# GeoMop/MLMC

Hardware: AMD Instinct MI355X
Metric: moment-evals/sec (samples x n_moments) (higher is better)
Workload: dtype f64

## Files before the change

### mlmc_amd/csrc/api.hip

```cpp
#include <cmath>
#include <chrono>
#include <cstring>
#include <new>

#include "common.hpp"
#include <algorithm>
#include <map>
#include <tuple>

namespace mlmc {

static thread_local std::string g_err;
void set_error(const std::string &msg) { g_err = msg; }
int fail(const std::string &msg) {
    g_err = msg;
    return 1;
}
Runtime &rt() {
    static Runtime r;
    return r;
}
std::recursive_mutex &api_mutex() {
    static std::recursive_mutex m;
    return m;
// ... 596 lines not shown
    return rc;
}

int mlmc_accum_create(const mlmc_basis *b, int32_t n_levels, int32_t mode, int32_t n_comp, mlmc_accum **out) {
    MLMC_API_GUARD;
    if (need_runtime()) return 1;
    if (!b || !out) return fail("mlmc_accum_create: null argument");
    if (n_levels <= 0 || n_comp <= 0) return fail("mlmc_accum_create: n_levels and n_comp must be > 0");
    const bool mean_only = (mode & MLMC_MODE_MEAN_ONLY) != 0;
    mode &= ~MLMC_MODE_MEAN_ONLY;
    if (mode != MLMC_MODE_MOMENTS && mode != MLMC_MODE_COV) return fail("mlmc_accum_create: unknown mode");
    mlmc_accum *a = new (std::nothrow) mlmc_accum();
    if (!a) return fail("out of memory");
    a->basis = b;
    a->n_levels = n_levels;
    a->mode = mode;
    const bool spline_band = mode == MLMC_MODE_COV && mean_only && b->out_size == 0 && b->p.kind == MLMC_SPLINE && b->p.size <= SPLINE_BAND_MAX_R;
    a->cov_from_values = mode == MLMC_MODE_COV && (b->out_size > 0 || (b->p.size > 128 && !spline_band));
    a->mean_only = mean_only && ((mode == MLMC_MODE_COV && !a->cov_from_values) || (mode == MLMC_MODE_MOMENTS && b->out_size > 0));
    a->mean_only_plain = mean_only && mode == MLMC_MODE_MOMENTS && b->out_size == 0 &&
                         (b->p.kind == MLMC_LEGENDRE || b->p.kind == MLMC_MONOMIAL || b->p.kind == KIND_CHEBYSHEV) && b->p.size > 64 &&
                         b->p.size <= 256;
    a->n_comp = n_comp;
    a->R = b->p.size;
    a->Rout = b->out_size > 0 ? b->out_size : b->p.size;
    a->RP = (((mode == MLMC_MODE_COV && b->out_size > 0 ? a->Rout : a->R) + 15) / 16) * 16;
    if (mode == MLMC_MODE_MOMENTS) {
        a->K = (int64_t)n_comp * a->Rout;
        a->int_width = 2 * (int64_t)a->R + (b->out_size > 0 ? (int64_t)a->RP * a->RP : 0);
    } else {
        a->K = (int64_t)n_comp * a->Rout * a->Rout;
        a->int_width = 3 * (int64_t)a->RP * a->RP;
    }
    const size_t tot = (size_t)n_levels * n_comp * a->int_width;
    a->state_bytes = sizeof(double) * tot + sizeof(int64_t) * 2 * n_levels;
    a->out_bytes = (sizeof(int64_t) + sizeof(double)) * 2 * n_levels + 2 * sizeof(double) * (size_t)n_levels * a->K;
    if (hipMalloc(&a->d_state, a->state_bytes) != hipSuccess || hipMalloc(&a->d_out, a->out_bytes) != hipSuccess ||
        hipHostMalloc(&a->h_out, a->out_bytes, hipHostMallocDefault) != hipSuccess) {
        mlmc_accum_destroy(a);
        return fail("mlmc_accum_create: device / pinned allocation failed");
    }
    a->d_totals = (double *)a->d_state;
    a->d_counts = (int64_t *)(a->d_totals + tot);
    a->level_flushed.assign(n_levels, 0);
    if (mode == MLMC_MODE_MOMENTS && n_comp == 1 && b->out_size == 0) {
        void *dev_view = nullptr;
// ... 11 lines not shown
    if (mode == MLMC_MODE_COV && !mean_only && !a->cov_from_values && b->out_size == 0 && b->p.size > lin_min_size() && b->p.size <= 128 &&
        (b->p.kind == MLMC_LEGENDRE || b->p.kind == MLMC_MONOMIAL) && b->p.is_clip &&
        std::fabs(b->p.ref0) <= 1.0 && std::fabs(b->p.ref1) <= 1.0 &&
        linearize_enabled()) {
        a->lin_eligible = true;
        const char *min_n = std::getenv("MLMC_HIP_LINEARIZE_MIN_N");
        a->lin_min_n = min_n ? std::atoll(min_n) : (a->R > 32 ? 100000 : 1500000);
        const char *lin0_env = std::getenv("MLMC_HIP_LINEARIZE_LEVEL0");
        a->lin0_eligible = a->R <= 64 && !(lin0_env && lin0_env[0] == '0');
        a->lin_cheb = b->p.kind == MLMC_LEGENDRE && linearize_chebyshev_enabled() && std::getenv("MLMC_HIP_NO_SPLIT") == nullptr;
        a->cov_rows = a->lin_cheb && a->lin0_eligible && a->R >= 49 && a->R <= 64 && a->RP == 64 && linearize_rowsums_enabled() &&
                      cov_rows_available();
    }
    *out = a;
    return mlmc_accum_reset(a);
}

int mlmc_accum_reset(mlmc_accum *a) {
    MLMC_API_GUARD;
    if (need_runtime()) return 1;
    if (!a) return fail("mlmc_accum_reset: null argument");
    hipStream_t st = rt().stream;
    a->pending.clear();
    std::fill(a->level_flushed.begin(), a->level_flushed.end(), 0);
    MLMC_HIP_CHECK(hipMemsetAsync(a->d_state, 0, a->state_bytes, st));
    if (a->xcov) {
        MLMC_HIP_CHECK(hipMemcpyAsync(a->d_shift, a->shift_host.data(), sizeof(double) * a->shift_host.size(), hipMemcpyHostToDevice, st));
        a->xcov_pushes = 0;
    }
    a->lin_used = a->lin0_used = false;
    if (a->d_rowsums) MLMC_HIP_CHECK(hipMemsetAsync(a->d_rowsums, 0, sizeof(double) * 64 * (size_t)a->n_levels * a->n_comp, st));
    a->lin_levels.assign(a->n_levels, 0);
    a->lin0_levels.assign(a->n_levels, 0);
    if (a->lin0)
        if (int rc = mlmc_accum_reset(a->lin0)) return rc;
    if (a->lin) return mlmc_accum_reset(a->lin);
    return 0;
}

void mlmc_accum_destroy(mlmc_accum *a) {
    MLMC_API_GUARD;
    if (!a) return;
    if (rt().ready) (void)wait_stream(rt().stream);
    if (a->lin) mlmc_accum_destroy(a->lin);
    if (a->lin_basis) mlmc_basis_destroy(a->lin_basis);
    if (a->lin0) mlmc_accum_destroy(a->lin0);
    if (a->lin0_basis) mlmc_basis_destroy(a->lin0_basis);
    void *ptrs[] = {a->d_state, a->d_partials, a->d_pcounts, a->d_stage_f, a->d_stage_c, a->d_mask, a->d_out, a->d_vals_f, a->d_vals_c, a->d_vals_tmp,
                    a->d_shift, a->d_rowparts, a->d_rowsums};
    for (void *p : ptrs)
        if (p) (void)hipFree(p);
    if (a->h_out) (void)hipHostFree(a->h_out);
    for (hipEvent_t e : a->ev) (void)hipEventDestroy(e);
    delete a;
}

int mlmc_accum_push(mlmc_accum *a, int32_t level, const double *fine, const double *coarse, int64_t n, int mem_kind) {
    MLMC_API_GUARD;
    if (need_runtime()) return 1;
    if (!a) return fail("mlmc_accum_push: null argument");
    if (level < 0 || level >= a->n_levels) return fail("mlmc_accum_push: level out of range");
    if (n < 0) return fail("mlmc_accum_push: negative n");
    if (n == 0) return 0;
    if (!fine) return fail("mlmc_accum_push: fine is NULL");
    if (n > ((int64_t)1 << 40)) return fail("mlmc_accum_push: chunk too large, split it");
    hipStream_t st = rt().stream;
    const size_t bytes = sizeof(double) * (size_t)n * a->n_comp;
    const double *d_f = fine, *d_c = coarse;
    if (mem_kind == MLMC_HOST) {
        if (bytes > a->stage_cap) {
            MLMC_HIP_CHECK(wait_stream(st));
            if (a->d_stage_f) (void)hipFree(a->d_stage_f);
            if (a->d_stage_c) (void)hipFree(a->d_stage_c);
            a->d_stage_f = a->d_stage_c = nullptr;
// ... 348 lines not shown
```

### mlmc_amd/csrc/common.hpp

```cpp
#pragma once
#include <hip/hip_runtime.h>
#include <stdint.h>
#include <mutex>
#include <string>
#include <vector>

#include "../../include/mlmc_hip.h"

namespace mlmc {

constexpr int WAVE = 64;
constexpr int ACC_THREADS = 256;
#ifndef MLMC_TERMS_PER_PASS
#define MLMC_TERMS_PER_PASS 64
#endif
constexpr int MAX_TERMS_PER_PASS = MLMC_TERMS_PER_PASS;
constexpr int KIND_CHEBYSHEV = 16;
static_assert(KIND_CHEBYSHEV > MLMC_SPLINE && KIND_CHEBYSHEV > MLMC_IDENTITY && KIND_CHEBYSHEV > MLMC_FOURIER && KIND_CHEBYSHEV > MLMC_MONOMIAL &&
                  KIND_CHEBYSHEV > MLMC_LEGENDRE && KIND_CHEBYSHEV > 7,
              "KIND_CHEBYSHEV must not collide with a public basis kind of mlmc_hip.h");
constexpr int SPLINE_BAND_MAX_R = 256;

void set_error(const std::string &msg);
int fail(const std::string &msg);
#define MLMC_HIP_CHECK(expr)                                                                   \
    do {                                                                                       \
        hipError_t _e = (expr);                                                                \
        if (_e != hipSuccess)                                                                  \
            return ::mlmc::fail(std::string(#expr) + ": " + hipGetErrorString(_e));            \
    } while (0)

std::recursive_mutex &api_mutex();
void bind_thread_to_device();
struct ApiGuard {
    std::lock_guard<std::recursive_mutex> lock;
    ApiGuard() : lock(api_mutex()) { bind_thread_to_device(); }
};
#define MLMC_API_GUARD ::mlmc::ApiGuard mlmc_api_guard_

struct Runtime {
    bool ready = false;
    int device = -1;
    int flags = 0;
// ... 31 lines not shown
    const uint64_t p0 = (uint64_t)0xD2511F53u * c[0], p1 = (uint64_t)0xCD9E8D57u * c[2];
    const uint32_t n0 = (uint32_t)(p1 >> 32) ^ c[1] ^ k0, n1 = (uint32_t)p1;
    const uint32_t n2 = (uint32_t)(p0 >> 32) ^ c[3] ^ k1, n3 = (uint32_t)p0;
    c[0] = n0; c[1] = n1; c[2] = n2; c[3] = n3;
}

struct BasisParams {
    int kind;
    int size;
    double shift, scale, ref0, ref1;
    int is_log, is_clip;
    double x_lo, x_hi;
};

}

struct mlmc_basis {
    mlmc::BasisParams p;
    int out_size = 0;
    std::vector<double> matrix;
    std::vector<double> scale_c;
    double *d_scale = nullptr;
    double *d_matrix = nullptr;
};

struct PendingSeg {
    const double *fine, *coarse;
    const uint8_t *mask;
    int64_t n;
    int level, comp;
    bool count;
};

struct mlmc_accum {
    const mlmc_basis *basis = nullptr;
    int n_levels = 0, mode = 0, n_comp = 1;
    bool mean_only = false;
    bool cov_from_values = false;
    bool mean_only_plain = false;
    int R = 0;
    int Rout = 0;
    int64_t K = 0;
    int64_t int_width = 0;
    void *d_state = nullptr;
    size_t state_bytes = 0;
    double *d_totals = nullptr;
    int64_t *d_counts = nullptr;
    double *d_partials = nullptr; size_t partials_cap = 0;
    int64_t *d_pcounts = nullptr; size_t pcounts_cap = 0;
    double *d_stage_f = nullptr, *d_stage_c = nullptr; size_t stage_cap = 0;
    uint8_t *d_mask = nullptr; size_t mask_cap = 0;
    double *d_vals_f = nullptr, *d_vals_c = nullptr; size_t vals_cap = 0;
    double *d_vals_tmp = nullptr; size_t vals_tmp_cap = 0;
    void *d_out = nullptr;
    size_t out_bytes = 0;
    void *h_out = nullptr;
    bool host_outputs = false;
    double *packed_target = nullptr;
    double *h_out_s = nullptr, *h_out_sp = nullptr; int64_t *h_out_n = nullptr;
    std::vector<char> level_flushed;
    double *d_out_s = nullptr, *d_out_sp = nullptr, *d_out_nd = nullptr; int64_t *d_out_n = nullptr;
    std::vector<hipEvent_t> ev;
    size_t ev_used = 0;
    double ms_total = 0;
    int64_t launches = 0, alg_bytes = 0;
    int64_t mfma_flops = 0;
    int RP = 0;
    bool lin_eligible = false, lin0_eligible = false;
    mlmc_accum *lin = nullptr;
    mlmc_basis *lin_basis = nullptr;
    double *d_lin_prod = nullptr;
    int lin_K = 0;
// ... 10 lines not shown
    bool cov_rows = false;
    double *d_rowparts = nullptr; size_t rowparts_cap = 0;
    double *d_rowsums = nullptr;
    double *d_conn = nullptr;
    int first_term = 0;
    std::vector<PendingSeg> pending;
    bool xcov = false;
    double *d_shift = nullptr;
    std::vector<double> shift_host;
    int64_t xcov_pushes = 0;
};

namespace mlmc {
int launch_eval(const mlmc_basis *b, const double *d_x, int64_t n, int size, double *d_out, double *scratch = nullptr);
int launch_eval_scaled_base(const mlmc_basis *b, const double *d_x, int64_t n, double *d_out);
int launch_mask(const mlmc_accum *a, const double *d_f, const double *d_c, int64_t n, uint8_t *d_mask, int64_t *d_counts_level);
int launch_moments_accum(mlmc_accum *a, int level, int comp, const double *d_f, const double *d_c, const uint8_t *d_mask,
                         int64_t n, bool count, bool defer);
int flush_moments(mlmc_accum *a);
int launch_moments_finalize(mlmc_accum *a);
int launch_cov_accum(mlmc_accum *a, int level, int comp, const double *d_f, const double *d_c, const uint8_t *d_mask,
                     int64_t n, bool count, int gram_mode, int ncomp = 1);
int launch_cov_finalize(mlmc_accum *a);
bool cov_rows_available();
constexpr int XCOV_MAX_M = 1024;
constexpr int MODE_XCOV = 2;
int launch_xcov_push(mlmc_accum *a, int level, const double *d_f, const double *d_c, int64_t n);
int launch_xcov_finalize(mlmc_accum *a);
bool product_table(int kind, int R, std::vector<double> &out);
bool square_product_table(int kind, int R, std::vector<double> &out);
bool product_table_chebyshev(int R, std::vector<double> &out);
bool square_product_table_chebyshev(int R, std::vector<double> &out);
int launch_cov_from_values(mlmc_accum *a, int level, int comp, const double *d_vf, const double *d_vc, const uint8_t *d_mask,
                           int64_t n, bool count, int gram_mode = 0);
int ensure(void **p, size_t *cap, size_t bytes);
void gauss_legendre(int n, std::vector<double> &x, std::vector<double> &w);
std::vector<double> effective_coeffs(const mlmc_basis *b, const double *lambda, const double *sigma, int R1);
int timing_begin(mlmc_accum *a);
int timing_end(mlmc_accum *a);
}
```

### mlmc_amd/csrc/cov.hip

```cpp
#include <cstring>

#include "device_basis.hpp"

namespace mlmc {

typedef double v4f64 __attribute__((ext_vector_type(4)));
#ifdef MLMC_PROF_COV
__device__ unsigned long long *g_prof_cov;
#define MLMC_COV_STAMP(slot)                                      \
    {                                                             \
        const unsigned long long now_ = __builtin_amdgcn_s_memtime(); \
        prof_acc[slot] += now_ - prof_t;                          \
        prof_t = now_;                                            \
    }
#else
#define MLMC_COV_STAMP(slot)
#endif
#ifndef MLMC_COV_PRIO_MFMA
#define MLMC_COV_PRIO_MFMA 0
#define MLMC_COV_PRIO_EVAL 2
#endif
#ifndef MLMC_COV_SLICE_BITS
#define MLMC_COV_SLICE_BITS 17
#endif
// ... 684 lines not shown
#define MLMC_COV_HAVE_ROWS 1
template <int KIND>
__global__ __launch_bounds__(256, COV_T4_WGS) void k_cov_accum_t4_rows(BasisParams bp, const double *__restrict__ fine,
                                                              const double *__restrict__ coarse, const uint8_t *__restrict__ mask,
                                                              int64_t n, double *__restrict__ partials,
                                                              int64_t *__restrict__ pcounts, double *__restrict__ rowparts) {
    __shared__ __attribute__((aligned(16))) double lds_f[64 * (COV_T4_BATCH + MLMC_COV_B128_PAD)];
    __shared__ __attribute__((aligned(16))) double lds_c[64 * (COV_T4_BATCH + MLMC_COV_B128_PAD)];
    __shared__ int ldc[2][2];
    fine += (int64_t)blockIdx.y * n;
    coarse += (int64_t)blockIdx.y * n;
    partials += (int64_t)blockIdx.y * gridDim.x * (cov_ng(3) * 64 * 64);
    rowparts += (int64_t)blockIdx.y * gridDim.x * 64;
    if (blockIdx.y) pcounts = nullptr;
    switch (__builtin_amdgcn_readfirstlane((int)(threadIdx.x >> 6))) {
        case 0: cov_t4_body<KIND, true, 3, 0, 0, true>(bp, fine, coarse, mask, n, partials, pcounts, lds_f, lds_c, ldc, rowparts); break;
        case 1: cov_t4_body<KIND, true, 3, 0, 1, true>(bp, fine, coarse, mask, n, partials, pcounts, lds_f, lds_c, ldc, rowparts); break;
        case 2: cov_t4_body<KIND, true, 3, 0, 2, true>(bp, fine, coarse, mask, n, partials, pcounts, lds_f, lds_c, ldc, rowparts); break;
        default: cov_t4_body<KIND, true, 3, 0, 3, true>(bp, fine, coarse, mask, n, partials, pcounts, lds_f, lds_c, ldc, rowparts); break;
    }
}
#endif

__global__ __launch_bounds__(1024) void k_reduce_cov(const double *__restrict__ partials, int nrows, int NT, int NG, int RP,
                                                    int roff, int coff, double *__restrict__ totals, int64_t comp_stride,
                                                    int mirror, const int64_t *__restrict__ pcounts, int nblocks,
                                                    int64_t *__restrict__ counts, const double *__restrict__ rowparts = nullptr,
                                                    double *__restrict__ rowsums = nullptr) {
    __shared__ double lds[64][17];
    const int c = threadIdx.x & 15, g = threadIdx.x >> 4;
    const int width = NG * NT * NT;
    const int n_col_groups = (width + 15) / 16;
    if (rowparts && (int)blockIdx.x >= n_col_groups && (int)blockIdx.x < n_col_groups + 4) {
        const int col = ((int)blockIdx.x - n_col_groups) * 16 + c;
        rowparts += (int64_t)blockIdx.y * nrows * 64;
        double acc = 0.0;
        for (int b = g; b < nrows; b += 64) acc += rowparts[(int64_t)b * 64 + col];
        lds[g][c] = acc;
        __syncthreads();
        if (g == 0) {
            double v = 0.0;
#pragma unroll
            for (int k = 0; k < 64; ++k) v += lds[k][c];
            rowsums[(int64_t)blockIdx.y * 64 + col] += v;
        }
        return;
    }
    if (pcounts && blockIdx.x == gridDim.x - 1) {
        if (blockIdx.y == 0 && threadIdx.x < 64) {
            int64_t a = 0, b = 0;
            for (int i = threadIdx.x; i < nblocks; i += 64) { a += pcounts[2 * i]; b += pcounts[2 * i + 1]; }
            for (int off = 32; off >= 1; off >>= 1) { a += __shfl_xor(a, off, 64); b += __shfl_xor(b, off, 64); }
            if (threadIdx.x == 0) { counts[0] += a; counts[1] += b; }
        }
        return;
    }
    partials += (int64_t)blockIdx.y * nrows * width;
    totals += (int64_t)blockIdx.y * comp_stride;
    const int col = blockIdx.x * 16 + c;
    double acc = 0.0;
    if (col < width)
        for (int b = g; b < nrows; b += 64) acc += partials[(int64_t)b * width + col];
    lds[g][c] = acc;
    __syncthreads();
    if (g == 0 && col < width) {
        double v = 0.0;
#pragma unroll
        for (int k = 0; k < 64; ++k) v += lds[k][c];
        const int gi = col / (NT * NT), rem = col % (NT * NT);
        const int row = roff + rem / NT, cc = coff + rem % NT;
        if (row < RP && cc < RP) {
            totals[(int64_t)gi * RP * RP + (int64_t)row * RP + cc] += v;
            if (mirror) totals[(int64_t)gi * RP * RP + (int64_t)cc * RP + row] += v;
        }
    }
}

template <int KIND, int T, int MODE, int BI, int BJ>
static int launch_cov_t(const BasisParams &bp, bool pair, int blocks, int ncomp, const double *d_f, const double *d_c,
                        const uint8_t *d_mask, int64_t n, int R, double *partials, int64_t *pcounts) {
    hipStream_t st = rt().stream;
    if constexpr (T == 4 && BI == BJ) {
        if (pair)
            hipLaunchKernelGGL((k_cov_accum_t4<KIND, true, MODE, BI>), dim3(blocks, ncomp), dim3(256), 0, st, bp, d_f, d_c, d_mask, n, R, partials, pcounts);
        else
            hipLaunchKernelGGL((k_cov_accum_t4<KIND, false, MODE, BI>), dim3(blocks, ncomp), dim3(256), 0, st, bp, d_f, d_c, d_mask, n, R, partials, pcounts);
    } else {
        if (pair)
            hipLaunchKernelGGL((k_cov_accum<KIND, T, true, MODE, BI, BJ>), dim3(blocks, ncomp), dim3(256), 0, st, bp, d_f, d_c, d_mask, n, R, partials, pcounts, 0, 0);
        else
            hipLaunchKernelGGL((k_cov_accum<KIND, T, false, MODE, BI, BJ>), dim3(blocks, ncomp), dim3(256), 0, st, bp, d_f, d_c, d_mask, n, R, partials, pcounts, 0, 0);
    }
    MLMC_HIP_CHECK(hipGetLastError());
    return 0;
}

template <int KIND, int MODE>
static int launch_cov_kind(const BasisParams &bp, int T, int bi, int bj, bool pair, int blocks, int ncomp, const double *d_f,
// ... 12 lines not shown
int launch_cov_from_values(mlmc_accum *a, int level, int comp, const double *d_vf, const double *d_vc, const uint8_t *d_mask,
                           int64_t n, bool count, int gram_mode) {
    if (n == 0) return 0;
    const bool diff_gram = gram_mode == 1;
    const int R = diff_gram ? a->R : a->Rout;
    hipStream_t st = rt().stream;
    const int T = (R <= 16) ? 1 : (R <= 32 ? 2 : 4);
    const int NT = 16 * T, NSL = 4 / T;
    const bool pair = d_vc != nullptr;
    const int NB = (R + 63) / 64;
    const int64_t n_batches = (n + COV_BATCH - 1) / COV_BATCH;
    const int NG = diff_gram ? 1 : 3;
    const size_t width = (size_t)NG * NT * NT;
    const BasisParams &bp = a->basis->p;
    double *totals = a->d_totals + ((int64_t)level * a->n_comp + comp) * a->int_width + (diff_gram ? 2 * (int64_t)R : 0);
    const bool symmetric = !pair || diff_gram;
    for (int bi = 0; bi < NB; ++bi)
        for (int bj = 0; bj < NB; ++bj) {
            if (symmetric && bj < bi) continue;
            const bool wide = bi != bj;
            int blocks = rt().n_cu * (wide ? 1 : 2);
            if (n_batches < blocks) blocks = (int)n_batches;
            const int n_slices = T <= 2 ? 4 : NSL;
            if (int rc = ensure((void **)&a->d_partials, &a->partials_cap, sizeof(double) * (size_t)blocks * n_slices * width)) return rc;
            if (int rc = ensure((void **)&a->d_pcounts, &a->pcounts_cap, sizeof(int64_t) * (size_t)blocks * 2)) return rc;
            const bool do_count = count && bi == 0 && bj == 0 && !diff_gram;
            int64_t *pc = do_count ? a->d_pcounts : nullptr;
            if (int rc = timing_begin(a)) return rc;
#define MLMC_COV_VALS1(TT, BJJ, MODE)                                                                                           \
    do {                                                                                                                        \
        if (pair)                                                                                                               \
            hipLaunchKernelGGL((k_cov_accum<MLMC_IDENTITY, TT, true, MODE, 0, BJJ, true>), dim3(blocks), dim3(256), 0, st, bp,      \
                               d_vf, d_vc, d_mask, n, R, a->d_partials, pc, 64 * bi, 64 * bj);                                  \
        else                                                                                                                    \
            hipLaunchKernelGGL((k_cov_accum<MLMC_IDENTITY, TT, false, MODE, 0, BJJ, true>), dim3(blocks), dim3(256), 0, st, bp,     \
                               d_vf, d_vc, d_mask, n, R, a->d_partials, pc, 64 * bi, 64 * bj);                                  \
    } while (0)
#define MLMC_COV_VALS(TT, BJJ)                                                                                                  \
    do {                                                                                                                        \
        if (diff_gram) MLMC_COV_VALS1(TT, BJJ, 1); else MLMC_COV_VALS1(TT, BJJ, 0);                                             \
    } while (0)
            if (T == 1) MLMC_COV_VALS(1, 0);
            else if (T == 2) MLMC_COV_VALS(2, 0);
            else if (!wide) MLMC_COV_VALS(4, 0);
            else MLMC_COV_VALS(4, 1);
#undef MLMC_COV_VALS
#undef MLMC_COV_VALS1
            MLMC_HIP_CHECK(hipGetLastError());
            if (int rc = timing_end(a)) return rc;
            if (!diff_gram) {
                a->launches += 1;
                a->alg_bytes += (int64_t)n * (pair ? 16 : 8);
                a->mfma_flops += (int64_t)512 * n * (T <= 2 ? (pair ? 2 * T * T + T * (T + 1) / 2 : T * (T + 1)) : (pair ? 3 : 2) * 16);
            }
            hipLaunchKernelGGL(k_reduce_cov, dim3((unsigned)((width + 15) / 16) + (do_count ? 1u : 0u)), dim3(1024), 0, st, a->d_partials,
                               blocks * n_slices, NT, NG, a->RP, 64 * bi, 64 * bj, totals, (int64_t)0, (symmetric && wide) ? 1 : 0,
                               do_count ? a->d_pcounts : (const int64_t *)nullptr, blocks, a->d_counts + 2 * (int64_t)level);
            MLMC_HIP_CHECK(hipGetLastError());
        }
    return 0;
}

constexpr int BAND_W = 5;
template <bool PAIR>
__global__ __launch_bounds__(256) void k_spline_band_accum(BasisParams bp, const double *__restrict__ fine,
                                                          const double *__restrict__ coarse, const uint8_t *__restrict__ mask,
                                                          int64_t n, int R, double *__restrict__ partials,
                                                          int64_t *__restrict__ pcounts) {
    extern __shared__ double band_tab[];
    __shared__ int ldc[4][2];
    const int RP8 = R + 8;
    fine += (int64_t)blockIdx.y * n;
    if (PAIR) coarse += (int64_t)blockIdx.y * n;
    partials += (int64_t)blockIdx.y * gridDim.x * (BAND_W * R);
    if (blockIdx.y) pcounts = nullptr;
    const int lane = threadIdx.x & 63, wave = threadIdx.x >> 6;
    for (int i = threadIdx.x; i < 4 * RP8 * BAND_W; i += 256) band_tab[i] = 0.0;
    __syncthreads();
    double *__restrict__ tab = band_tab + (size_t)wave * RP8 * BAND_W;
    int n_keep = 0, n_rm = 0;
    const int64_t T = (int64_t)gridDim.x * 256;
// ... 83 lines not shown
    __syncthreads();
    if (g == 0 && col < width) {
        double v = 0.0;
#pragma unroll
        for (int k = 0; k < 64; ++k) v += lds[k][c];
        const int r = col / BAND_W, w = col % BAND_W;
        if (r >= 1) {
            if (w == 4) {
                totals[r] += v;
                totals[(int64_t)r * RP] += v;
            } else if (r + w < R) {
                totals[(int64_t)r * RP + r + w] += v;
                if (w) totals[(int64_t)(r + w) * RP + r] += v;
            }
        }
    }
}

static int launch_spline_band(mlmc_accum *a, int level, int comp, const double *d_f, const double *d_c, const uint8_t *d_mask, int64_t n,
                              bool count, int ncomp) {
    hipStream_t st = rt().stream;
    const int R = a->R;
    const bool pair = d_c != nullptr;
    int blocks = rt().n_cu * 4;
    const int64_t want = (n + 255) / 256;
    if (want < blocks) blocks = (int)want;
    if (int rc = ensure((void **)&a->d_partials, &a->partials_cap, sizeof(double) * (size_t)blocks * BAND_W * R * ncomp)) return rc;
    if (int rc = ensure((void **)&a->d_pcounts, &a->pcounts_cap, sizeof(int64_t) * (size_t)blocks * 2)) return rc;
    const size_t lds = sizeof(double) * 4 * (size_t)(R + 8) * BAND_W;
    const BasisParams &bp = a->basis->p;
    double *totals = a->d_totals + ((int64_t)level * a->n_comp + comp) * a->int_width;
    if (int rc = timing_begin(a)) return rc;
    if (pair)
        hipLaunchKernelGGL(k_spline_band_accum<true>, dim3(blocks, ncomp), dim3(256), lds, st, bp, d_f, d_c, d_mask, n, R, a->d_partials, a->d_pcounts);
    else
        hipLaunchKernelGGL(k_spline_band_accum<false>, dim3(blocks, ncomp), dim3(256), lds, st, bp, d_f, d_c, d_mask, n, R, a->d_partials, a->d_pcounts);
    MLMC_HIP_CHECK(hipGetLastError());
    if (int rc = timing_end(a)) return rc;
    a->launches += 1;
    a->alg_bytes += (int64_t)n * (pair ? 16 : 8) * ncomp;
    hipLaunchKernelGGL(k_reduce_band, dim3((BAND_W * R + 15) / 16 + 1, ncomp), dim3(1024), 0, st, a->d_partials, a->d_pcounts, blocks, R, a->RP,
                       totals, a->int_width, count ? a->d_counts + 2 * (int64_t)level : (int64_t *)nullptr, pair ? 0 : 1);
    MLMC_HIP_CHECK(hipGetLastError());
    return 0;
}

// ... 21 lines not shown
    const int R = a->R;
    if (a->basis->p.kind == MLMC_SPLINE && gram_mode == 2 && R <= SPLINE_BAND_MAX_R)
        return launch_spline_band(a, level, comp, d_f, d_c, d_mask, n, count, ncomp);
    if (R > 128) return fail("covariance accumulation in registers covers 128 moments; larger bases go through launch_cov_from_values");
    hipStream_t st = rt().stream;
    const int T = (R <= 16) ? 1 : (R <= 32 ? 2 : 4);
    const int NT = 16 * T, NSL = 4 / T;
    const int NB = (R + 63) / 64;
    const bool pair = d_c != nullptr;
    const int64_t bsz = T == 4 ? (pair ? COV_T4_BATCH : 2 * COV_T4_BATCH) : cov_batch(T, false, false, pair);
    const int64_t n_batches = (n + bsz - 1) / bsz;
    const BasisParams &bp = a->basis->p;
    double *totals0 = a->d_totals + ((int64_t)level * a->n_comp + comp) * a->int_width + (diff_gram_only ? 2 * (int64_t)R : 0);
    for (int bi = 0; bi < NB; ++bi)
        for (int bj = 0; bj < NB; ++bj) {
            if (!pair && bj < bi) continue;
            const bool two_slots = gram_mode == 3 && T == 4 && bi == bj;
            const int NG = gram_mode == 3 ? (two_slots ? 2 : 3) : cov_ng(gram_mode);
            const size_t width = (size_t)NG * NT * NT;
            double *totals = totals0 + (two_slots ? (int64_t)a->RP * a->RP : 0);
            int blocks = rt().n_cu * ((bi != bj) ? ((pair && MLMC_COV_WIDE_BATCH < 64) ? 2 : 1) : (T == 1 ? 4 : (T == 4 ? COV_T4_WGS : 2)));
            if ((n_batches + 3) / 4 < blocks) blocks = (int)((n_batches + 3) / 4);
            const int n_slices = T <= 2 ? 4 : NSL;
            if (int rc = ensure((void **)&a->d_partials, &a->partials_cap, sizeof(double) * (size_t)blocks * n_slices * width * ncomp)) return rc;
            if (int rc = ensure((void **)&a->d_pcounts, &a->pcounts_cap, sizeof(int64_t) * (size_t)blocks * 2)) return rc;
            const bool do_count = count && bi == 0 && bj == 0;
            int64_t *pc = do_count ? a->d_pcounts : nullptr;
            const bool timed = !diff_gram_only;
            if (timed) if (int rc = timing_begin(a)) return rc;
            int rc;
#define MLMC_COV_DISPATCH(KIND)                                                                                               \
    rc = gram_mode == 3 ? launch_cov_kind<KIND, 3>(bp, T, bi, bj, pair, blocks, ncomp, d_f, d_c, d_mask, n, R, a->d_partials, pc) \
       : gram_mode == 2 ? launch_cov_kind<KIND, 2>(bp, T, bi, bj, pair, blocks, ncomp, d_f, d_c, d_mask, n, R, a->d_partials, pc) \
       : diff_gram_only ? launch_cov_kind<KIND, 1>(bp, T, bi, bj, pair, blocks, ncomp, d_f, d_c, d_mask, n, R, a->d_partials, pc) \
                        : launch_cov_kind<KIND, 0>(bp, T, bi, bj, pair, blocks, ncomp, d_f, d_c, d_mask, n, R, a->d_partials, pc)
#define MLMC_COV_DISPATCH012(KIND)                                                                                            \
    rc = gram_mode == 2 ? launch_cov_kind<KIND, 2>(bp, T, bi, bj, pair, blocks, ncomp, d_f, d_c, d_mask, n, R, a->d_partials, pc) \
       : diff_gram_only ? launch_cov_kind<KIND, 1>(bp, T, bi, bj, pair, blocks, ncomp, d_f, d_c, d_mask, n, R, a->d_partials, pc) \
                        : launch_cov_kind<KIND, 0>(bp, T, bi, bj, pair, blocks, ncomp, d_f, d_c, d_mask, n, R, a->d_partials, pc)
            if (gram_mode == 3 && bp.kind != MLMC_LEGENDRE && bp.kind != MLMC_MONOMIAL)
                return fail("covariance: the variance-only pass exists for the polynomial families");
            const bool rows = a->cov_rows && gram_mode == 3 && pair;
            if (rows) {
#ifdef MLMC_COV_HAVE_ROWS
                if (int rce = ensure((void **)&a->d_rowparts, &a->rowparts_cap, sizeof(double) * (size_t)blocks * 64 * ncomp)) return rce;
                hipLaunchKernelGGL((k_cov_accum_t4_rows<MLMC_LEGENDRE>), dim3(blocks, ncomp), dim3(256), 0, st, bp, d_f, d_c, d_mask, n, a->d_partials, pc, a->d_rowparts);
                MLMC_HIP_CHECK(hipGetLastError());
                rc = 0;
#else
                return fail("covariance: this build has no row sums in the matrix kernel");
#endif
            } else
            switch (bp.kind) {
                case MLMC_LEGENDRE: MLMC_COV_DISPATCH(MLMC_LEGENDRE); break;
                case MLMC_MONOMIAL: MLMC_COV_DISPATCH(MLMC_MONOMIAL); break;
                case MLMC_FOURIER: MLMC_COV_DISPATCH012(MLMC_FOURIER); break;
                case MLMC_SPLINE: MLMC_COV_DISPATCH012(MLMC_SPLINE); break;
                default: return fail("covariance: unsupported basis kind");
            }
#undef MLMC_COV_DISPATCH
#undef MLMC_COV_DISPATCH012
            if (rc) return rc;
            if (timed) {
                if (int rc2 = timing_end(a)) return rc2;
                a->launches += 1;
                a->alg_bytes += (int64_t)n * (pair ? 16 : 8) * ncomp;
                a->mfma_flops += (int64_t)512 * cov_tiles_per_sample(T, bi == bj, pair, gram_mode) * n * ncomp;
            }
            hipLaunchKernelGGL(k_reduce_cov, dim3((unsigned)((width + 15) / 16) + (rows ? 4u : 0u) + (do_count ? 1u : 0u), ncomp), dim3(1024), 0, st, a->d_partials,
                               blocks * n_slices, NT, NG, a->RP, 64 * bi, 64 * bj, totals, a->int_width, (!pair && bi != bj) ? 1 : 0,
                               do_count ? a->d_pcounts : (const int64_t *)nullptr, blocks, a->d_counts + 2 * (int64_t)level,
                               rows ? a->d_rowparts : (const double *)nullptr,
                               rows ? a->d_rowsums + ((int64_t)level * a->n_comp + comp) * 64 : (double *)nullptr);
            MLMC_HIP_CHECK(hipGetLastError());
        }
    return 0;
}

__global__ void k_cov_finalize(const double *__restrict__ totals, const double *__restrict__ scale_c, int R, int RP,
                               int64_t int_width, double *__restrict__ out_s, double *__restrict__ out_sp,
                               const int64_t *__restrict__ counts, int n_levels, int64_t *__restrict__ out_n,
                               double *__restrict__ out_nd, int mean_only, const int64_t *__restrict__ counts2) {
    const int lc = blockIdx.y;
    if (lc == 0 && blockIdx.x == 0)
        for (int l = threadIdx.x; l < n_levels; l += blockDim.x) {
            const int64_t kept = counts[2 * l] + (counts2 ? counts2[2 * l] : 0), removed = counts[2 * l + 1] + (counts2 ? counts2[2 * l + 1] : 0);
            out_n[l] = kept;
            out_n[n_levels + l] = removed;
            out_nd[l] = (double)kept;
            out_nd[n_levels + l] = (double)removed;
        }
    const double *G0 = totals + (int64_t)lc * int_width;
    const double *G1 = G0 + (int64_t)RP * RP;
    const double *G2 = G1 + (int64_t)RP * RP;
    const int idx = blockIdx.x * blockDim.x + threadIdx.x;
    if (idx >= R * R) return;
    const int i = idx / R, j = idx % R;
// ... 44 lines not shown
                    v = sr.scale[k] * sr.totals[(int64_t)jb.row[l] * sr.width + k];
                }
            }
            m_s[q] = v;
        }
        __syncthreads();
        if (idx < RR) {
            double acc[LIN_LC];
#pragma unroll
            for (int l = 0; l < LIN_LC; ++l) acc[l] = 0.0;
            const int k0 = (parity_step == 2 && !sr.squares) ? ((idx / R + idx % R) & 1) : 0;
            for (int k = k0; k < K; k += parity_step) {
                const double c = sr.prod[(int64_t)k * RR + idx];
#pragma unroll
                for (int l = 0; l < LIN_LC; ++l) acc[l] = __builtin_fma(c, m_s[l * K + k], acc[l]);
            }
#pragma unroll
            for (int l = 0; l < LIN_LC; ++l)
                if (l < jb.n_rows) jb.out[(int64_t)jb.row[l] * RR + idx] += acc[l];
        }
    }
}

int launch_cov_finalize(mlmc_accum *a) {
    if (a->lin && a->lin_used) {
        if (int rc = flush_moments(a->lin)) return rc;
    }
    const bool lin0 = a->lin0 && a->lin0_used;
    if (lin0) {
        if (int rc = flush_moments(a->lin0)) return rc;
    }
    const int pstep = a->basis->p.kind == MLMC_LEGENDRE ? 2 : 1;
    const int n_lc = a->n_levels * a->n_comp;
    const bool vals = a->cov_from_values;
    const int R = vals ? a->Rout : a->R;
    hipLaunchKernelGGL(k_cov_finalize, dim3((R * R + 255) / 256, n_lc), dim3(256), 0, rt().stream, a->d_totals,
                       vals ? (const double *)nullptr : a->basis->d_scale, R,
                       a->RP, a->int_width, a->d_out_s, a->d_out_sp, a->d_counts, a->n_levels, a->d_out_n, a->d_out_nd,
                       a->mean_only ? 1 : 0, lin0 ? a->lin0->d_counts : (const int64_t *)nullptr);
    MLMC_HIP_CHECK(hipGetLastError());
    const bool lin = a->lin && a->lin_used;
    if (!lin && !lin0) return 0;
    LinSrc src0, src02, src1;
    std::memset(&src0, 0, sizeof(src0));
    std::memset(&src02, 0, sizeof(src02));
    std::memset(&src1, 0, sizeof(src1));
    int max_K = 0;
    if (lin0) {
        src0.prod = a->d_lin0_prod1; src0.totals = a->lin0->d_totals; src0.scale = a->lin0_basis->d_scale;
        src0.width = a->lin0->int_width; src0.K = a->lin_K; src0.squares = 0;
        src02 = src0;
        src02.prod = a->d_lin0_prod; src02.K = a->lin0_K; src02.squares = 1;
        max_K = a->lin0_K;
    }
    if (lin) {
        src1.prod = a->d_lin_prod; src1.totals = a->lin->d_totals; src1.scale = a->lin_basis->d_scale;
        src1.width = a->lin->int_width; src1.K = a->lin_K; src1.squares = 0;
        if (a->cov_rows) { src1.rowsums = a->d_rowsums; src1.conn = a->d_conn; src1.pscale = a->d_conn + 64 * 64; }
        if (a->lin_K > max_K) max_K = a->lin_K;
    }
    LinJobs jobs;
    std::memset(&jobs, 0, sizeof(jobs));
    int n_jobs = 0;
    const dim3 block(256);
    auto launch = [&]() -> int {
        if (n_jobs == 0) return 0;
        hipLaunchKernelGGL(k_cov_lin_mean, dim3((R * R + 255) / 256, n_jobs), block, sizeof(double) * LIN_LC * max_K, rt().stream, jobs, R, pstep);
        MLMC_HIP_CHECK(hipGetLastError());
        std::memset(&jobs, 0, sizeof(jobs));
        n_jobs = 0;
        return 0;
    };
    for (int cls = 1; cls <= 4; ++cls) {
        LinJob *jb = nullptr;
        for (int lc = 0; lc < n_lc; ++lc) {
            const int level = lc / a->n_comp;
            const int fed = ((lin0 && a->lin0_levels[level]) ? 1 : 0) | ((lin && a->lin_levels[level]) ? 2 : 0);
            if (cls <= 3 ? fed != cls : !(fed & 1)) continue;
            if (!jb || jb->n_rows == LIN_LC) {
                if (n_jobs == LIN_MAX_JOBS)
                    if (int rc = launch()) return rc;
                jb = &jobs.job[n_jobs++];
                jb->out = cls == 4 ? a->d_out_sp : a->d_out_s;
                jb->src[0] = cls == 4 ? src02 : (cls == 2 ? src1 : src0);
                if (cls == 3) jb->src[1] = src1;
            }
            jb->row[jb->n_rows++] = lc;
        }
    }
    return launch();
// ... 4 lines not shown
```

Before: 319.8 billion.

## Batch covariance partial reductions across pushes and widen linear mean kernel

Covariance reduction launches are deferred into a pending table with per-slot partial buffers, so that up to several reductions, from different levels and tiles, run in one k_reduce_cov launch with a chain grid dimension. This is meant to cut per-push kernel launch overhead and small-grid underutilisation. It also adds a 64-thread k_cov_lin_mean_wide finalize kernel that prefetches products, giving more blocks and more memory-level parallelism. The cost is extra device memory for the slots, more complex flush ordering, and a risk of same-level conflicts, which are handled with chains and by flushing when a level's pair status differs.

New measurement: 318.9 billion (median of 2 runs). Within noise of the previous version (-0.3%).

```diff
diff --git a/mlmc_amd/csrc/api.hip b/mlmc_amd/csrc/api.hip
--- a/mlmc_amd/csrc/api.hip
+++ b/mlmc_amd/csrc/api.hip
@@ -642,6 +642,11 @@
                          (b->p.kind == MLMC_LEGENDRE || b->p.kind == MLMC_MONOMIAL || b->p.kind == KIND_CHEBYSHEV) && b->p.size > 64 &&
                          b->p.size <= 256;
     a->n_comp = n_comp;
+    if (mode == MLMC_MODE_COV) {
+        const char *pend = std::getenv("MLMC_HIP_COV_PENDING");
+        const int want = pend ? std::atoi(pend) : COV_PENDING_DEFAULT;
+        a->cov_pend_cap = want < 1 ? 1 : (want > COV_PENDING_MAX ? COV_PENDING_MAX : want);
+    }
     a->R = b->p.size;
     a->Rout = b->out_size > 0 ? b->out_size : b->p.size;
     a->RP = (((mode == MLMC_MODE_COV && b->out_size > 0 ? a->Rout : a->R) + 15) / 16) * 16;
@@ -699,6 +704,8 @@
     if (!a) return fail("mlmc_accum_reset: null argument");
     hipStream_t st = rt().stream;
     a->pending.clear();
+    a->cov_pend.n = 0;
+    a->cov_pend_bytes = 0;
     std::fill(a->level_flushed.begin(), a->level_flushed.end(), 0);
     MLMC_HIP_CHECK(hipMemsetAsync(a->d_state, 0, a->state_bytes, st));
     if (a->xcov) {
@@ -727,6 +734,9 @@
                     a->d_shift, a->d_rowparts, a->d_rowsums};
     for (void *p : ptrs)
         if (p) (void)hipFree(p);
+    for (CovSlot &sl : a->cov_slot)
+        for (void *p : {(void *)sl.d_partials, (void *)sl.d_pcounts, (void *)sl.d_rowparts})
+            if (p) (void)hipFree(p);
     if (a->h_out) (void)hipHostFree(a->h_out);
     for (hipEvent_t e : a->ev) (void)hipEventDestroy(e);
     delete a;
diff --git a/mlmc_amd/csrc/common.hpp b/mlmc_amd/csrc/common.hpp
--- a/mlmc_amd/csrc/common.hpp
+++ b/mlmc_amd/csrc/common.hpp
@@ -19,6 +19,9 @@
 static_assert(KIND_CHEBYSHEV > MLMC_SPLINE && KIND_CHEBYSHEV > MLMC_IDENTITY && KIND_CHEBYSHEV > MLMC_FOURIER && KIND_CHEBYSHEV > MLMC_MONOMIAL &&
                   KIND_CHEBYSHEV > MLMC_LEGENDRE && KIND_CHEBYSHEV > 7,
               "KIND_CHEBYSHEV must not collide with a public basis kind of mlmc_hip.h");
+constexpr int COV_PENDING_MAX = 8;
+constexpr int COV_PENDING_DEFAULT = 4;
+constexpr size_t COV_PENDING_MAX_BYTES = (size_t)512 << 20;
 constexpr int SPLINE_BAND_MAX_R = 256;
 
 void set_error(const std::string &msg);
@@ -96,6 +99,29 @@
     std::vector<double> scale_c;
     double *d_scale = nullptr;
     double *d_matrix = nullptr;
+};
+
+struct CovSlot {
+    double *d_partials = nullptr; size_t partials_cap = 0;
+    int64_t *d_pcounts = nullptr; size_t pcounts_cap = 0;
+    double *d_rowparts = nullptr; size_t rowparts_cap = 0;
+};
+struct CovRedDesc {
+    const double *partials;
+    const int64_t *pcounts;
+    const double *rowparts;
+    double *totals;
+    int64_t *counts;
+    double *rowsums;
+    int64_t comp_stride;
+    int nrows, nblocks, NG, goff;
+    int bi, bj, mirror, ncomp;
+    int level, pair, chain;
+};
+struct CovRedTable {
+    CovRedDesc d[mlmc::COV_PENDING_MAX];
+    int blk[mlmc::COV_PENDING_MAX];
+    int n, n_blk, NT;
 };
 
 struct PendingSeg {
@@ -122,6 +148,10 @@
     int64_t *d_counts = nullptr;
     double *d_partials = nullptr; size_t partials_cap = 0;
     int64_t *d_pcounts = nullptr; size_t pcounts_cap = 0;
+    CovSlot cov_slot[mlmc::COV_PENDING_MAX - 1];
+    CovRedTable cov_pend = {};
+    int cov_pend_cap = 1;
+    size_t cov_pend_bytes = 0;
     double *d_stage_f = nullptr, *d_stage_c = nullptr; size_t stage_cap = 0;
     uint8_t *d_mask = nullptr; size_t mask_cap = 0;
     double *d_vals_f = nullptr, *d_vals_c = nullptr; size_t vals_cap = 0;
@@ -178,6 +208,7 @@
 int launch_cov_accum(mlmc_accum *a, int level, int comp, const double *d_f, const double *d_c, const uint8_t *d_mask,
                      int64_t n, bool count, int gram_mode, int ncomp = 1);
 int launch_cov_finalize(mlmc_accum *a);
+int cov_reduce_flush(mlmc_accum *a);
 bool cov_rows_available();
 constexpr int XCOV_MAX_M = 1024;
 constexpr int MODE_XCOV = 2;
diff --git a/mlmc_amd/csrc/cov.hip b/mlmc_amd/csrc/cov.hip
--- a/mlmc_amd/csrc/cov.hip
+++ b/mlmc_amd/csrc/cov.hip
@@ -730,58 +730,118 @@
 }
 #endif
 
-__global__ __launch_bounds__(1024) void k_reduce_cov(const double *__restrict__ partials, int nrows, int NT, int NG, int RP,
-                                                    int roff, int coff, double *__restrict__ totals, int64_t comp_stride,
-                                                    int mirror, const int64_t *__restrict__ pcounts, int nblocks,
-                                                    int64_t *__restrict__ counts, const double *__restrict__ rowparts = nullptr,
-                                                    double *__restrict__ rowsums = nullptr) {
+__global__ __launch_bounds__(1024) void k_reduce_cov(CovRedTable tab, int NT, int RP) {
     __shared__ double lds[64][17];
     const int c = threadIdx.x & 15, g = threadIdx.x >> 4;
-    const int width = NG * NT * NT;
-    const int n_col_groups = (width + 15) / 16;
-    if (rowparts && (int)blockIdx.x >= n_col_groups && (int)blockIdx.x < n_col_groups + 4) {
-        const int col = ((int)blockIdx.x - n_col_groups) * 16 + c;
-        rowparts += (int64_t)blockIdx.y * nrows * 64;
-        double acc = 0.0;
-        for (int b = g; b < nrows; b += 64) acc += rowparts[(int64_t)b * 64 + col];
-        lds[g][c] = acc;
+    const int gpg = NT * NT / 16;
+    const int n_tile_items = tab.n_blk * 3 * gpg;
+    const int item = blockIdx.x;
+    for (int q = 0; q < tab.n; ++q) {
+        const CovRedDesc &d = tab.d[q];
+        if (d.chain != (int)blockIdx.z || (int)blockIdx.y >= d.ncomp) continue;
+        const int nrows = d.nrows;
+        if (item >= n_tile_items + 4) {
+            if (!d.pcounts) continue;
+            if (blockIdx.y == 0 && threadIdx.x < 64) {
+                int64_t a = 0, b = 0;
+                for (int i = threadIdx.x; i < d.nblocks; i += 64) { a += d.pcounts[2 * i]; b += d.pcounts[2 * i + 1]; }
+                for (int off = 32; off >= 1; off >>= 1) { a += __shfl_xor(a, off, 64); b += __shfl_xor(b, off, 64); }
+                if (threadIdx.x == 0) { d.counts[0] += a; d.counts[1] += b; }
+            }
+        } else if (item >= n_tile_items) {
+            if (!d.rowparts) continue;
+            const int col = (item - n_tile_items) * 16 + c;
+            const double *__restrict__ rowparts = d.rowparts + (int64_t)blockIdx.y * d.nblocks * 64;
+            double acc = 0.0;
+            for (int b = g; b < d.nblocks; b += 64) acc += rowparts[(int64_t)b * 64 + col];
+            lds[g][c] = acc;
+            __syncthreads();
+            if (g == 0) {
+                double v = 0.0;
+#pragma unroll
+                for (int k = 0; k < 64; ++k) v += lds[k][c];
+                d.rowsums[(int64_t)blockIdx.y * 64 + col] += v;
+            }
+        } else {
+            if (tab.blk[item / (3 * gpg)] != d.bi * 256 + d.bj) continue;
+            const int lcg = item % (3 * gpg) - d.goff * gpg;
+            if (lcg < 0 || lcg >= d.NG * gpg) continue;
+            const int width = d.NG * NT * NT;
+            const double *__restrict__ partials = d.partials + (int64_t)blockIdx.y * nrows * width;
+            double *__restrict__ totals = d.totals + (int64_t)blockIdx.y * d.comp_stride;
+            const int col = lcg * 16 + c;
+            double acc = 0.0;
+            for (int b = g; b < nrows; b += 64) acc += partials[(int64_t)b * width + col];
+            lds[g][c] = acc;
+            __syncthreads();
+            if (g == 0) {
+                double v = 0.0;
+#pragma unroll
+                for (int k = 0; k < 64; ++k) v += lds[k][c];
+                const int gi = col / (NT * NT), rem = col % (NT * NT);
+                const int row = 64 * d.bi + rem / NT, cc = 64 * d.bj + rem % NT;
+                if (row < RP && cc < RP) {
+                    totals[(int64_t)gi * RP * RP + (int64_t)row * RP + cc] += v;
+                    if (d.mirror) totals[(int64_t)gi * RP * RP + (int64_t)cc * RP + row] += v;
+                }
+            }
+        }
         __syncthreads();
-        if (g == 0) {
-            double v = 0.0;
-#pragma unroll
-            for (int k = 0; k < 64; ++k) v += lds[k][c];
-            rowsums[(int64_t)blockIdx.y * 64 + col] += v;
-        }
-        return;
-    }
-    if (pcounts && blockIdx.x == gridDim.x - 1) {
-        if (blockIdx.y == 0 && threadIdx.x < 64) {
-            int64_t a = 0, b = 0;
-            for (int i = threadIdx.x; i < nblocks; i += 64) { a += pcounts[2 * i]; b += pcounts[2 * i + 1]; }
-            for (int off = 32; off >= 1; off >>= 1) { a += __shfl_xor(a, off, 64); b += __shfl_xor(b, off, 64); }
-            if (threadIdx.x == 0) { counts[0] += a; counts[1] += b; }
-        }
-        return;
-    }
-    partials += (int64_t)blockIdx.y * nrows * width;
-    totals += (int64_t)blockIdx.y * comp_stride;
-    const int col = blockIdx.x * 16 + c;
-    double acc = 0.0;
-    if (col < width)
-        for (int b = g; b < nrows; b += 64) acc += partials[(int64_t)b * width + col];
-    lds[g][c] = acc;
-    __syncthreads();
-    if (g == 0 && col < width) {
-        double v = 0.0;
-#pragma unroll
-        for (int k = 0; k < 64; ++k) v += lds[k][c];
-        const int gi = col / (NT * NT), rem = col % (NT * NT);
-        const int row = roff + rem / NT, cc = coff + rem % NT;
-        if (row < RP && cc < RP) {
-            totals[(int64_t)gi * RP * RP + (int64_t)row * RP + cc] += v;
-            if (mirror) totals[(int64_t)gi * RP * RP + (int64_t)cc * RP + row] += v;
-        }
-    }
+    }
+}
+
+struct CovSlotRef {
+    double *&partials; size_t &partials_cap;
+    int64_t *&pcounts; size_t &pcounts_cap;
+    double *&rowparts; size_t &rowparts_cap;
+};
+static CovSlotRef cov_slot_ref(mlmc_accum *a, int i) {
+    if (i == 0) return {a->d_partials, a->partials_cap, a->d_pcounts, a->pcounts_cap, a->d_rowparts, a->rowparts_cap};
+    CovSlot &s = a->cov_slot[i - 1];
+    return {s.d_partials, s.partials_cap, s.d_pcounts, s.pcounts_cap, s.d_rowparts, s.rowparts_cap};
+}
+static int cov_slot_begin(mlmc_accum *a, int level, bool pair, size_t partial_bytes, int *slot) {
+    CovRedTable &t = a->cov_pend;
+    bool flush = t.n >= a->cov_pend_cap || (t.n > 0 && a->cov_pend_bytes + partial_bytes > COV_PENDING_MAX_BYTES);
+    for (int q = 0; q < t.n && !flush; ++q) flush = t.d[q].level == level && (t.d[q].pair != 0) != pair;
+    if (flush)
+        if (int rc = cov_reduce_flush(a)) return rc;
+    *slot = t.n;
+    return 0;
+}
+
+static int cov_slot_end(mlmc_accum *a, const CovRedDesc &d, int NT, size_t partial_bytes, bool now) {
+    CovRedTable &t = a->cov_pend;
+    t.d[t.n++] = d;
+    t.NT = NT;
+    a->cov_pend_bytes += partial_bytes;
+    if (now || t.n >= a->cov_pend_cap) return cov_reduce_flush(a);
+    return 0;
+}
+
+int cov_reduce_flush(mlmc_accum *a) {
+    CovRedTable &t = a->cov_pend;
+    if (t.n == 0) return 0;
+    int n_chains = 0, max_comp = 1;
+    t.n_blk = 0;
+    for (int q = 0; q < t.n; ++q) {
+        int ch = -1;
+        for (int p = 0; p < q && ch < 0; ++p)
+            if (t.d[p].level == t.d[q].level) ch = t.d[p].chain;
+        t.d[q].chain = ch < 0 ? n_chains++ : ch;
+        const int blk = t.d[q].bi * 256 + t.d[q].bj;
+        int k = 0;
+        while (k < t.n_blk && t.blk[k] != blk) ++k;
+        if (k == t.n_blk) t.blk[t.n_blk++] = blk;
+        if (t.d[q].ncomp > max_comp) max_comp = t.d[q].ncomp;
+    }
+    const int NT = t.NT;
+    hipLaunchKernelGGL(k_reduce_cov, dim3((unsigned)(t.n_blk * 3 * (NT * NT / 16) + 5), (unsigned)max_comp, (unsigned)n_chains), dim3(1024), 0,
+                       rt().stream, t, NT, a->RP);
+    t.n = 0;
+    a->cov_pend_bytes = 0;
+    MLMC_HIP_CHECK(hipGetLastError());
+    return 0;
 }
 
 template <int KIND, int T, int MODE, int BI, int BJ>
@@ -840,7 +900,9 @@
             int blocks = rt().n_cu * (wide ? 1 : 2);
             if (n_batches < blocks) blocks = (int)n_batches;
             const int n_slices = T <= 2 ? 4 : NSL;
-            if (int rc = ensure((void **)&a->d_partials, &a->partials_cap, sizeof(double) * (size_t)blocks * n_slices * width)) return rc;
+            const size_t pbytes = sizeof(double) * (size_t)blocks * n_slices * width;
+            if (int rc = cov_reduce_flush(a)) return rc;
+            if (int rc = ensure((void **)&a->d_partials, &a->partials_cap, pbytes)) return rc;
             if (int rc = ensure((void **)&a->d_pcounts, &a->pcounts_cap, sizeof(int64_t) * (size_t)blocks * 2)) return rc;
             const bool do_count = count && bi == 0 && bj == 0 && !diff_gram;
             int64_t *pc = do_count ? a->d_pcounts : nullptr;
@@ -871,10 +933,12 @@
                 a->alg_bytes += (int64_t)n * (pair ? 16 : 8);
                 a->mfma_flops += (int64_t)512 * n * (T <= 2 ? (pair ? 2 * T * T + T * (T + 1) / 2 : T * (T + 1)) : (pair ? 3 : 2) * 16);
             }
-            hipLaunchKernelGGL(k_reduce_cov, dim3((unsigned)((width + 15) / 16) + (do_count ? 1u : 0u)), dim3(1024), 0, st, a->d_partials,
-                               blocks * n_slices, NT, NG, a->RP, 64 * bi, 64 * bj, totals, (int64_t)0, (symmetric && wide) ? 1 : 0,
-                               do_count ? a->d_pcounts : (const int64_t *)nullptr, blocks, a->d_counts + 2 * (int64_t)level);
-            MLMC_HIP_CHECK(hipGetLastError());
+            CovRedDesc rd;
+            std::memset(&rd, 0, sizeof(rd));
+            rd.partials = a->d_partials; rd.pcounts = pc; rd.totals = totals; rd.counts = a->d_counts + 2 * (int64_t)level;
+            rd.nrows = blocks * n_slices; rd.nblocks = blocks; rd.NG = NG; rd.bi = bi; rd.bj = bj; rd.mirror = (symmetric && wide) ? 1 : 0;
+            rd.ncomp = 1; rd.level = level; rd.pair = pair ? 1 : 0;
+            if (int rc = cov_slot_end(a, rd, NT, pbytes, true)) return rc;
         }
     return 0;
 }
@@ -1004,6 +1068,7 @@
     hipStream_t st = rt().stream;
     const int R = a->R;
     const bool pair = d_c != nullptr;
+    if (int rc = cov_reduce_flush(a)) return rc;
     int blocks = rt().n_cu * 4;
     const int64_t want = (n + 255) / 256;
     if (want < blocks) blocks = (int)want;
@@ -1071,29 +1136,34 @@
             int blocks = rt().n_cu * ((bi != bj) ? ((pair && MLMC_COV_WIDE_BATCH < 64) ? 2 : 1) : (T == 1 ? 4 : (T == 4 ? COV_T4_WGS : 2)));
             if ((n_batches + 3) / 4 < blocks) blocks = (int)((n_batches + 3) / 4);
             const int n_slices = T <= 2 ? 4 : NSL;
-            if (int rc = ensure((void **)&a->d_partials, &a->partials_cap, sizeof(double) * (size_t)blocks * n_slices * width * ncomp)) return rc;
-            if (int rc = ensure((void **)&a->d_pcounts, &a->pcounts_cap, sizeof(int64_t) * (size_t)blocks * 2)) return rc;
+            const size_t pbytes = sizeof(double) * (size_t)blocks * n_slices * width * ncomp;
+            int slot_i = 0;
+            if (int rc = cov_slot_begin(a, level, pair, pbytes, &slot_i)) return rc;
+            const CovSlotRef slot = cov_slot_ref(a, slot_i);
+            if (int rc = ensure((void **)&slot.partials, &slot.partials_cap, pbytes)) return rc;
+            if (int rc = ensure((void **)&slot.pcounts, &slot.pcounts_cap, sizeof(int64_t) * (size_t)blocks * 2)) return rc;
+            double *const d_part = slot.partials;
             const bool do_count = count && bi == 0 && bj == 0;
-            int64_t *pc = do_count ? a->d_pcounts : nullptr;
+            int64_t *pc = do_count ? slot.pcounts : nullptr;
             const bool timed = !diff_gram_only;
             if (timed) if (int rc = timing_begin(a)) return rc;
             int rc;
 #define MLMC_COV_DISPATCH(KIND)                                                                                               \
-    rc = gram_mode == 3 ? launch_cov_kind<KIND, 3>(bp, T, bi, bj, pair, blocks, ncomp, d_f, d_c, d_mask, n, R, a->d_partials, pc) \
-       : gram_mode == 2 ? launch_cov_kind<KIND, 2>(bp, T, bi, bj, pair, blocks, ncomp, d_f, d_c, d_mask, n, R, a->d_partials, pc) \
-       : diff_gram_only ? launch_cov_kind<KIND, 1>(bp, T, bi, bj, pair, blocks, ncomp, d_f, d_c, d_mask, n, R, a->d_partials, pc) \
-                        : launch_cov_kind<KIND, 0>(bp, T, bi, bj, pair, blocks, ncomp, d_f, d_c, d_mask, n, R, a->d_partials, pc)
+    rc = gram_mode == 3 ? launch_cov_kind<KIND, 3>(bp, T, bi, bj, pair, blocks, ncomp, d_f, d_c, d_mask, n, R, d_part, pc) \
+       : gram_mode == 2 ? launch_cov_kind<KIND, 2>(bp, T, bi, bj, pair, blocks, ncomp, d_f, d_c, d_mask, n, R, d_part, pc) \
+       : diff_gram_only ? launch_cov_kind<KIND, 1>(bp, T, bi, bj, pair, blocks, ncomp, d_f, d_c, d_mask, n, R, d_part, pc) \
+                        : launch_cov_kind<KIND, 0>(bp, T, bi, bj, pair, blocks, ncomp, d_f, d_c, d_mask, n, R, d_part, pc)
 #define MLMC_COV_DISPATCH012(KIND)                                                                                            \
-    rc = gram_mode == 2 ? launch_cov_kind<KIND, 2>(bp, T, bi, bj, pair, blocks, ncomp, d_f, d_c, d_mask, n, R, a->d_partials, pc) \
-       : diff_gram_only ? launch_cov_kind<KIND, 1>(bp, T, bi, bj, pair, blocks, ncomp, d_f, d_c, d_mask, n, R, a->d_partials, pc) \
-                        : launch_cov_kind<KIND, 0>(bp, T, bi, bj, pair, blocks, ncomp, d_f, d_c, d_mask, n, R, a->d_partials, pc)
+    rc = gram_mode == 2 ? launch_cov_kind<KIND, 2>(bp, T, bi, bj, pair, blocks, ncomp, d_f, d_c, d_mask, n, R, d_part, pc) \
+       : diff_gram_only ? launch_cov_kind<KIND, 1>(bp, T, bi, bj, pair, blocks, ncomp, d_f, d_c, d_mask, n, R, d_part, pc) \
+                        : launch_cov_kind<KIND, 0>(bp, T, bi, bj, pair, blocks, ncomp, d_f, d_c, d_mask, n, R, d_part, pc)
             if (gram_mode == 3 && bp.kind != MLMC_LEGENDRE && bp.kind != MLMC_MONOMIAL)
                 return fail("covariance: the variance-only pass exists for the polynomial families");
             const bool rows = a->cov_rows && gram_mode == 3 && pair;
             if (rows) {
 #ifdef MLMC_COV_HAVE_ROWS
-                if (int rce = ensure((void **)&a->d_rowparts, &a->rowparts_cap, sizeof(double) * (size_t)blocks * 64 * ncomp)) return rce;
-                hipLaunchKernelGGL((k_cov_accum_t4_rows<MLMC_LEGENDRE>), dim3(blocks, ncomp), dim3(256), 0, st, bp, d_f, d_c, d_mask, n, a->d_partials, pc, a->d_rowparts);
+                if (int rce = ensure((void **)&slot.rowparts, &slot.rowparts_cap, sizeof(double) * (size_t)blocks * 64 * ncomp)) return rce;
+                hipLaunchKernelGGL((k_cov_accum_t4_rows<MLMC_LEGENDRE>), dim3(blocks, ncomp), dim3(256), 0, st, bp, d_f, d_c, d_mask, n, d_part, pc, slot.rowparts);
                 MLMC_HIP_CHECK(hipGetLastError());
                 rc = 0;
 #else
@@ -1116,12 +1186,15 @@
                 a->alg_bytes += (int64_t)n * (pair ? 16 : 8) * ncomp;
                 a->mfma_flops += (int64_t)512 * cov_tiles_per_sample(T, bi == bj, pair, gram_mode) * n * ncomp;
             }
-            hipLaunchKernelGGL(k_reduce_cov, dim3((unsigned)((width + 15) / 16) + (rows ? 4u : 0u) + (do_count ? 1u : 0u), ncomp), dim3(1024), 0, st, a->d_partials,
-                               blocks * n_slices, NT, NG, a->RP, 64 * bi, 64 * bj, totals, a->int_width, (!pair && bi != bj) ? 1 : 0,
-                               do_count ? a->d_pcounts : (const int64_t *)nullptr, blocks, a->d_counts + 2 * (int64_t)level,
-                               rows ? a->d_rowparts : (const double *)nullptr,
-                               rows ? a->d_rowsums + ((int64_t)level * a->n_comp + comp) * 64 : (double *)nullptr);
-            MLMC_HIP_CHECK(hipGetLastError());
+            CovRedDesc rd;
+            std::memset(&rd, 0, sizeof(rd));
+            rd.partials = d_part; rd.pcounts = pc; rd.totals = totals; rd.counts = a->d_counts + 2 * (int64_t)level;
+            if (rows) { rd.rowparts = slot.rowparts; rd.rowsums = a->d_rowsums + ((int64_t)level * a->n_comp + comp) * 64; }
+            rd.comp_stride = a->int_width;
+            rd.nrows = blocks * n_slices; rd.nblocks = blocks; rd.NG = NG; rd.goff = two_slots ? 1 : 0;
+            rd.bi = bi; rd.bj = bj; rd.mirror = (!pair && bi != bj) ? 1 : 0;
+            rd.ncomp = ncomp; rd.level = level; rd.pair = pair ? 1 : 0;
+            if (int rc2 = cov_slot_end(a, rd, NT, pbytes, a->mode != MLMC_MODE_COV || diff_gram_only)) return rc2;
         }
     return 0;
 }
@@ -1212,7 +1285,89 @@
     }
 }
 
+constexpr int LIN_WIDE_THREADS = 64;
+constexpr int LIN_AHEAD = 16;
+__global__ __launch_bounds__(LIN_WIDE_THREADS) void k_cov_lin_mean_wide(LinJobs jobs, int R, int parity_step) {
+    extern __shared__ double m_s[];
+    __shared__ double p_s[LIN_LC][64];
+    const LinJob &jb = jobs.job[blockIdx.y];
+    const int idx = blockIdx.x * LIN_WIDE_THREADS + threadIdx.x;
+    const int RR = R * R;
+    const int n_rows = jb.n_rows;
+    for (int e = 0; e < 2; ++e) {
+        const LinSrc &sr = jb.src[e];
+        if (!sr.prod) continue;
+        const int K = sr.K;
+        __syncthreads();
+        if (sr.rowsums) {
+            for (int q = threadIdx.x; q < n_rows * 64; q += LIN_WIDE_THREADS)
+                p_s[q >> 6][q & 63] = sr.pscale[q & 63] * sr.rowsums[(int64_t)jb.row[q >> 6] * 64 + (q & 63)];
+            __syncthreads();
+        }
+        for (int k = threadIdx.x; k < K; k += LIN_WIDE_THREADS) {
+            double v[LIN_LC];
+#pragma unroll
+            for (int l = 0; l < LIN_LC; ++l) v[l] = 0.0;
+            if (sr.rowsums && k < 64) {
+                double cn[32];
+#pragma unroll
+                for (int u = 0; u < 32; ++u) cn[u] = sr.conn[k * 64 + (k & 1) + 2 * u];
+#pragma unroll
+                for (int u = 0; u < 32; ++u) {
+                    const int j = (k & 1) + 2 * u;
+                    if (j <= k) {
+#pragma unroll
+                        for (int l = 0; l < LIN_LC; ++l)
+                            if (l < n_rows) v[l] = __builtin_fma(cn[u], p_s[l][j], v[l]);
+                    }
+                }
+            } else {
+                const double sc = sr.scale[k];
+#pragma unroll
+                for (int l = 0; l < LIN_LC; ++l)
+                    if (l < n_rows) v[l] = sc * sr.totals[(int64_t)jb.row[l] * sr.width + k];
+            }
+#pragma unroll
+            for (int l = 0; l < LIN_LC; ++l) m_s[l * K + k] = v[l];
+        }
+        __syncthreads();
+        if (idx < RR) {
+            double acc[LIN_LC];
+#pragma unroll
+            for (int l = 0; l < LIN_LC; ++l) acc[l] = 0.0;
+            const int k0 = (parity_step == 2 && !sr.squares) ? ((idx / R + idx % R) & 1) : 0;
+            const double *__restrict__ pr = sr.prod + idx;
+            const int n_k = (K - k0 + parity_step - 1) / parity_step;
+            double c[LIN_AHEAD], cn[LIN_AHEAD];
+#pragma unroll
+            for (int u = 0; u < LIN_AHEAD; ++u) c[u] = pr[(int64_t)(k0 + (u < n_k ? u : (n_k > 0 ? n_k - 1 : 0)) * parity_step) * RR];
+            for (int t = 0; t < n_k; t += LIN_AHEAD) {
+#pragma unroll
+                for (int u = 0; u < LIN_AHEAD; ++u) {
+                    const int tn = t + LIN_AHEAD + u;
+                    cn[u] = pr[(int64_t)(k0 + (tn < n_k ? tn : n_k - 1) * parity_step) * RR];
+                }
+#pragma unroll
+                for (int u = 0; u < LIN_AHEAD; ++u) {
+                    const int k = k0 + (t + u) * parity_step;
+                    if (t + u < n_k) {
+#pragma unroll
+                        for (int l = 0; l < LIN_LC; ++l)
+                            if (l < n_rows) acc[l] = __builtin_fma(c[u], m_s[l * K + k], acc[l]);
+                    }
+                }
+#pragma unroll
+                for (int u = 0; u < LIN_AHEAD; ++u) c[u] = cn[u];
+            }
+#pragma unroll
+            for (int l = 0; l < LIN_LC; ++l)
+                if (l < n_rows) jb.out[(int64_t)jb.row[l] * RR + idx] += acc[l];
+        }
+    }
+}
+
 int launch_cov_finalize(mlmc_accum *a) {
+    if (int rc = cov_reduce_flush(a)) return rc;
     if (a->lin && a->lin_used) {
         if (int rc = flush_moments(a->lin)) return rc;
     }
@@ -1253,9 +1408,15 @@
     std::memset(&jobs, 0, sizeof(jobs));
     int n_jobs = 0;
     const dim3 block(256);
+    const char *wide_env = std::getenv("MLMC_HIP_LIN_MEAN_WIDE");
+    const bool wide = !(wide_env && wide_env[0] == '0');
     auto launch = [&]() -> int {
         if (n_jobs == 0) return 0;
-        hipLaunchKernelGGL(k_cov_lin_mean, dim3((R * R + 255) / 256, n_jobs), block, sizeof(double) * LIN_LC * max_K, rt().stream, jobs, R, pstep);
+        if (wide)
+            hipLaunchKernelGGL(k_cov_lin_mean_wide, dim3((R * R + LIN_WIDE_THREADS - 1) / LIN_WIDE_THREADS, n_jobs), dim3(LIN_WIDE_THREADS),
+                               sizeof(double) * LIN_LC * max_K, rt().stream, jobs, R, pstep);
+        else
+            hipLaunchKernelGGL(k_cov_lin_mean, dim3((R * R + 255) / 256, n_jobs), block, sizeof(double) * LIN_LC * max_K, rt().stream, jobs, R, pstep);
         MLMC_HIP_CHECK(hipGetLastError());
         std::memset(&jobs, 0, sizeof(jobs));
         n_jobs = 0;
```
